# dat-rohit/distributed-neural-network

Hardware: AMD Instinct MI355X
Metric: images/sec (whole node) + epoch time, CIFAR-10 CNN bs=64 at 1/2/4/8 MI355X (higher is better)
Workload: dtype bf16; 1 GPU; model=reference CIFAR-10 CNN (models/model.py Network, 62,006 params), engine=HipEngine, pipelined_step=True, persistent_launch=True, launch=direct-aql, global_batch=64, per_gpu_batch=64, parallelism=dp1, sync=step-allreduce, optimizer=SGD lr=0.001 momentum=0.9, every step, safe_transport=0

## Files before the change

csrc/kernels/lenet_fused.hip:

```cpp
#include <algorithm>
#include <cstddef>
#include <string>

#include "pers_common.h"
#include "runtime/aql_dispatch.h"

namespace dnn {

constexpr int NT = 512;
constexpr int CODES_PER_SAMPLE = 6 * 196 + 400;

constexpr int L_REGA = 0;
constexpr int L_REGA_SZ = 96256;
constexpr int L_REGB = L_REGA + L_REGA_SZ;
constexpr int L_REGB_SZ = 44544;
constexpr int B_WF = 17472;
constexpr int L_P1 = L_REGB + L_REGB_SZ;
constexpr int L_CODE1 = L_P1 + 3360;
constexpr int L_A0 = L_CODE1 + 1184;
constexpr int L_A0B = L_A0 + 1600;
constexpr int L_CODE2 = L_A0B + 832;
constexpr int L_H1 = L_CODE2 + 400;
constexpr int L_H1B = L_H1 + 512;
constexpr int L_H2 = L_H1B + 256;
constexpr int L_H2B = L_H2 + 384;
constexpr int L_LOG = L_H2B + 192;
constexpr int L_DZ3 = L_LOG + 64;
constexpr int L_DZ3B = L_DZ3 + 64;
constexpr int L_DZ2 = L_DZ3B + 64;
constexpr int L_DZ2B = L_DZ2 + 384;
constexpr int L_DZ1 = L_DZ2B + 192;
constexpr int L_DZ1B = L_DZ1 + 512;
constexpr int L_DA0 = L_DZ1B + 256;
constexpr int L_IMG = L_DA0 + 1600;
constexpr int L_MISC = L_IMG + 3072;
constexpr int L_F1C = L_MISC + 64;
constexpr int LDS_TOTAL = L_F1C + 128;
static_assert(LDS_TOTAL <= 163840, "LDS budget");
static_assert(B_WF + 20480 <= L_REGB_SZ, "REGB sub-layout");

constexpr int A_R3 = 0;
constexpr int A_DY2 = 73728;
constexpr int DY2_CS = 176;
constexpr int A_DP1 = A_DY2 + 16 * DY2_CS * 2;
constexpr int A_RS = A_DP1 + 4704;
constexpr int A_DY1 = 0;
constexpr int DY1_CH = 1824;
constexpr int A_RS1 = A_DY1 + 6 * DY1_CH;
static_assert(A_RS + 1152 <= L_REGA_SZ, "REGA sub-layout");
static_assert(A_RS1 + 672 <= A_DP1, "phase F scratch must not overlap dP1");

__device__ __forceinline__ bf16 u8norm_bf16(uint32_t u) {
  return (bf16)__builtin_fmaf((float)u, (float)(2.0 / 255.0), -1.0f);
}

__device__ __forceinline__ void lds_barrier() {
  asm volatile("s_waitcnt lgkmcnt(0)\n\ts_barrier" ::: "memory");
}

__device__ __forceinline__ void dma16(const void* gsrc, uint32_t lds_base) {
  unsigned keep;
  asm volatile(
      "s_mov_b32 %0, m0\n\ts_mov_b32 m0, %2\n\ts_nop 0\n\tglobal_load_lds_dwordx4 %1, off\n\ts_mov_b32 m0, %0"
      : "=&s"(keep)
      : "v"(gsrc), "s"(lds_base)
      : "memory");
}

__device__ __forceinline__ uint32_t lds_addr(const void* p) {
  return (uint32_t)(uintptr_t)(const __attribute__((address_space(3))) unsigned char*)p;
}

template <typename T>
__device__ __forceinline__ void consume(T& v) {
  asm volatile("" : "+v"(v));
}

__device__ __forceinline__ f32x4 mfma32(bf16x8 a, bf16x8 b, f32x4 c) {
  return __builtin_amdgcn_mfma_f32_16x16x32_bf16(a, b, c, 0, 0, 0);
}

__device__ __forceinline__ bf16x8 zero8() {
  bf16x8 z;
#pragma unroll
  for (int j = 0; j < 8; ++j) z[j] = (bf16)0.f;
  return z;
}

__device__ __forceinline__ bf16x8 row0(const bf16* x, int k0, int fr) {
  const bf16x8 v = *reinterpret_cast<const bf16x8*>(x + k0);
  return fr == 0 ? v : zero8();
}

__device__ __forceinline__ bf16x8 tr_frag(const bf16* m, int ld, int k0, int n0, int kmax, int lane) {
  typedef __attribute__((address_space(3))) bf16x4* lp;
  const int l16 = lane & 15, q = l16 >> 2, p = l16 & 3, fg = lane >> 4;
  const int r0 = min(k0 + 8 * fg + q, kmax - 1), r1 = min(k0 + 8 * fg + 4 + q, kmax - 1);
  const bf16x4 lo = __builtin_amdgcn_ds_read_tr16_b64_v4bf16((lp)(m + r0 * ld + n0 + 4 * p));
  const bf16x4 hi = __builtin_amdgcn_ds_read_tr16_b64_v4bf16((lp)(m + r1 * ld + n0 + 4 * p));
  bf16x8 v;
#pragma unroll
  for (int j = 0; j < 4; ++j) { v[j] = lo[j]; v[4 + j] = hi[j]; }
  return v;
}

__device__ __forceinline__ void build_r1_part(const uint8_t* img, bf16x8* R1, int row, int q) {
  const uint32_t* src = reinterpret_cast<const uint32_t*>(img + row * 32);
  uint32_t w[4];
#pragma unroll
  for (int k = 0; k < 4; ++k) w[k] = src[min(2 * q + k, 7)];
  bf16 v[16];
#pragma unroll
  for (int k = 0; k < 16; ++k) {
    const uint32_t u = (w[k >> 2] >> (8 * (k & 3))) & 0xffu;
    const bf16 t = u8norm_bf16(u);
    v[k] = (8 * q + k < 32) ? t : (bf16)0.f;
  }
#pragma unroll
  for (int x = 0; x < 8; ++x) {
    if (8 * q + x < 29) {
// ... 69 lines not shown
constexpr int PIPE_CTR_STRIDE = 32;
static_assert(PIPE_BLOCKS == GRAD_REDUCE_BLOCKS, "the pipelined launch runs the whole grad_reduce");
static_assert(PIPE_C2_BLOCKS > 0, "conv2 keeps blocks of its own");
int pipe_reduce_blocks() { return PIPE_BLOCKS; }
int pipe_groups() { return PIPE_GROUPS; }

__device__ __forceinline__ int pipe_group_blocks(int grp) {
  return grp == PG_C1 ? PIPE_C1_BLOCKS : grp == PG_C2 ? PIPE_C2_BLOCKS : PIPE_MLP_BLOCKS;
}
__device__ __forceinline__ long pipe_ctr_index(int par, int grp) { return (long)(PIPE_GROUPS * par + grp) * PIPE_CTR_STRIDE; }
__device__ __forceinline__ long pipe_flag_index(int par, int grp, int b, int batch) {
  return ((long)(PIPE_GROUPS * par + grp) * batch + b) * PIPE_CTR_STRIDE;
}

__device__ __forceinline__ void pipe_reduce(const ReduceArgs& a, const PipeCtl& pc, int wg, long long* stamps) {
  const int half = threadIdx.x >> 8, m = 2 * wg + half, rtid = threadIdx.x & 255;
  if (wg == 0) {
    if (threadIdx.x < PIPE_GROUPS) pc.ctr[pipe_ctr_index(pc.par ^ 1, threadIdx.x)] = 0u;
    for (int i = threadIdx.x; i < PIPE_GROUPS * a.batch; i += blockDim.x)
      pc.flg[pipe_flag_index(pc.par ^ 1, i / a.batch, i % a.batch, a.batch)] = 0u;
  }
  int grp = -1;
  if (m < pc.nred) {
    int rblk = 0;
    if (pc.nred > 1) {
      if (m < PIPE_CONV_BLOCKS) { rblk = PIPE_MLP_BLOCKS + m; grp = m < PIPE_C1_BLOCKS ? PG_C1 : PG_C2; }
      else if (m == PIPE_CONV_BLOCKS) rblk = PIPE_MLP_BLOCKS + PIPE_CONV_BLOCKS;
      else { rblk = m - PIPE_CONV_BLOCKS - 1; grp = PG_MLP; }
    }
    WtSink sk;
    grad_reduce_body(a, sk, rblk, rtid);
  }
  if (stamps != nullptr && threadIdx.x == 0) stamps[16 + 4 * wg + 1] = (long long)__builtin_amdgcn_s_memrealtime();
  asm volatile("s_waitcnt vmcnt(0)" ::: "memory");
  __syncthreads();
  if ((rtid >> 6) == 0 && grp >= 0) {
    unsigned old = 0;
    if (rtid == 0)
      old = __hip_atomic_fetch_add(pc.ctr + pipe_ctr_index(pc.par, grp), 1u, __ATOMIC_RELAXED, __HIP_MEMORY_SCOPE_AGENT);
    old = __builtin_amdgcn_readfirstlane(old);
    if (stamps != nullptr && rtid == 0 && half == 0) stamps[16 + 4 * wg + 3] = (long long)__builtin_amdgcn_s_memrealtime();
    if (old == (unsigned)pipe_group_blocks(grp) - 1u)
      for (int b = rtid; b < a.batch; b += 64)
        __hip_atomic_store(pc.flg + pipe_flag_index(pc.par, grp, b, a.batch), 1u, __ATOMIC_RELAXED,
                           __HIP_MEMORY_SCOPE_AGENT);
  }
}

__device__ __forceinline__ void pipe_wait(const PipeCtl& pc, int grp, int b, int batch, long long* diag = nullptr,
                                          int also = -1, bool* also_set = nullptr, unsigned tgt = 1u) {
  const unsigned* f = pc.flg + pipe_flag_index(pc.par, grp, b, batch);
  const unsigned* g = pc.flg + pipe_flag_index(pc.par, also < 0 ? grp : also, b, batch);
  if (__hip_atomic_load(pc.err, __ATOMIC_RELAXED, __HIP_MEMORY_SCOPE_AGENT) != 0u) return;
  const long long t0 = wall_clock64();
  if (diag != nullptr) diag[0] = t0;
  long long polls = 0;
  while (true) {
    const unsigned v = __hip_atomic_load(f, __ATOMIC_RELAXED, __HIP_MEMORY_SCOPE_AGENT);
    const unsigned w = also >= 0 ? __hip_atomic_load(g, __ATOMIC_RELAXED, __HIP_MEMORY_SCOPE_AGENT) : 0u;
    if (diag != nullptr && polls < 12) {
      diag[4082 + 2 * polls] = (long long)__builtin_amdgcn_s_memrealtime();
      diag[4083 + 2 * polls] = v;
    }
    if (v >= tgt) {
      if (also_set != nullptr) *also_set = w >= tgt;
      break;
    }
    ++polls;
    if (diag != nullptr) diag[1] = polls;
    __builtin_amdgcn_s_sleep(2);
    if (wall_clock64() - t0 > pc.timeout_ticks) {
      __hip_atomic_store(pc.err, 1u, __ATOMIC_RELAXED, __HIP_MEMORY_SCOPE_SYSTEM);
      break;
    }
  }
}

constexpr int PERS_WG = (PIPE_BLOCKS + 1) / 2;
constexpr int PERS_CONV_WG = (PIPE_CONV_BLOCKS + 1 + 1) / 2;
constexpr int PERS_C1_WG = PIPE_C1_BLOCKS / 2;
static_assert((PIPE_CONV_BLOCKS + 1) % 2 == 0, "conv + bookkeeping blocks fill whole workgroups");
static_assert(PIPE_C1_BLOCKS % 2 == 0, "the conv1 group is whole workgroups");
static_assert(PERS_WG <= PERS_RROW, "one ready word per reduction workgroup in a sample's row");
int persist_ctl_bytes(int batch) { return (int)(pers_arrive_off(batch) + (long)PERS_WG * PERS_AROW * 4); }

__device__ __forceinline__ void pers_arrive(const PipeCtl& pc, int kind, int b, unsigned tag, int lane) {
  const int w0 = kind ? PERS_CONV_WG : 0, nw = kind ? PERS_WG - PERS_CONV_WG : PERS_CONV_WG;
  if (lane < nw) st_tag(pc.arrive + (long)(w0 + lane) * PERS_AROW + b, tag);
}

struct PersPoll {
  unsigned err, v;
};
__device__ __forceinline__ const unsigned* pers_ready_word(const PipeCtl& pc, int b, int lane) {
  return pc.flg + (long)b * PERS_RROW + min(lane, PERS_WG - 1);
}
__device__ __forceinline__ PersPoll pers_poll_issue(const PipeCtl& pc, int b, int lane) {
  return PersPoll{ld_tag(pc.err), ld_tag(pers_ready_word(pc, b, lane))};
}
__device__ __forceinline__ void pers_wait_ready(const PipeCtl& pc, int b, int lo, int hi, unsigned tgt, int lane,
                                                int also_lo = 0, int also_hi = 0, bool* also_set = nullptr,
                                                long long* diag = nullptr, bool has_pre = false, unsigned pre_err = 0u,
                                                unsigned pre_v = 0u) {
  const unsigned* row = pers_ready_word(pc, b, lane);
  unsigned ferr = pre_err, v = pre_v;
  if (!has_pre) {
    const PersPoll first = pers_poll_issue(pc, b, lane);
    ferr = first.err;
    v = first.v;
  }
  if (ferr != 0u) return;
  const long long t0 = wall_clock64();
  if (diag != nullptr && lane == 0) diag[0] = t0;
  long long polls = 0;
  while (true) {
    if (__all((lane < lo || lane >= hi) || tag_ge(v, tgt))) {
      if (also_set != nullptr) *also_set = __all((lane < also_lo || lane >= also_hi) || tag_ge(v, tgt));
      break;
    }
    ++polls;
    if (diag != nullptr && lane == 0) diag[1] = polls;
    __builtin_amdgcn_s_sleep(1);
    if (wall_clock64() - t0 > pc.timeout_ticks) {
      if (lane == 0) __hip_atomic_store(pc.err, 1u, __ATOMIC_RELAXED, __HIP_MEMORY_SCOPE_SYSTEM);
      break;
    }
    v = ld_tag(row);
  }
}

template <class F>
__device__ __forceinline__ bool pers_wait_c1_early_fc1(const PipeCtl& pc, int b, unsigned tgt, int lane,
                                                       F&& stream_all) {
  const unsigned* row = pers_ready_word(pc, b, lane);
  const PersPoll first = pers_poll_issue(pc, b, lane);
  if (first.err != 0u) return false;
  const long long t0 = wall_clock64();
  bool streamed = false;
  unsigned v = first.v;
  while (true) {
    if (__all(lane >= PERS_C1_WG || tag_ge(v, tgt))) break;
    if (!streamed && __all(lane < PERS_CONV_WG || tag_ge(v, tgt))) {
      stream_all();
      streamed = true;
    }
    __builtin_amdgcn_s_sleep(1);
    if (wall_clock64() - t0 > pc.timeout_ticks) {
      if (lane == 0) __hip_atomic_store(pc.err, 1u, __ATOMIC_RELAXED, __HIP_MEMORY_SCOPE_SYSTEM);
      break;
    }
    v = ld_tag(row);
  }
  return streamed;
}

template <int XNR>
__device__ __forceinline__ void pers_reduce(const ReduceArgs& a, const PipeCtl& pc, int wg, long long* stamps) {
  const int half = __builtin_amdgcn_readfirstlane(threadIdx.x >> 8), m = 2 * wg + half, rtid = threadIdx.x & 255,
            lane = threadIdx.x & 63;
  const bool bk = m == PIPE_CONV_BLOCKS;
  int rblk = 0;
  if (m < PIPE_CONV_BLOCKS) rblk = PIPE_MLP_BLOCKS + m;
  else if (!bk) rblk = m - PIPE_CONV_BLOCKS - 1;
  const unsigned g0 = __builtin_amdgcn_readfirstlane(ld_tag(pc.gen + blockIdx.x));
  const int gb = bk ? PIPE_MLP_BLOCKS + PIPE_CONV_BLOCKS : rblk;
  const unsigned xc0 = XNR > 1 ? __builtin_amdgcn_readfirstlane(a.xp_ctr[gb]) : 0u;
  if (bk && rtid < 64) bookkeeping_pers(a, pc, lane, -1);
  const unsigned* arr = pc.arrive + (long)wg * PERS_AROW;
  for (int t = 0; t < pc.nsteps; ++t) {
    if (threadIdx.x < 64) pers_wait_rows(pc, arr, a.batch, g0 + (unsigned)t + 1u, lane);
    const bool st = stamps != nullptr && threadIdx.x == 0 && t == pc.nsteps - 1;
    if (st) stamps[2400 + 4 * wg] = (long long)__builtin_amdgcn_s_memrealtime();
    __syncthreads();
    int tid_o = threadIdx.x;
    asm volatile("" : "+v"(tid_o));
    const int rtid_s = tid_o & 255;
    if (bk) {
      if (rtid < 64) bookkeeping_pers(a, pc, lane, t);
    } else if constexpr (XNR > 1) {
      const unsigned step = xc0 + (unsigned)t + 1u;
      const bool failed = __hip_atomic_load(a.xp_err, __ATOMIC_RELAXED, __HIP_MEMORY_SCOPE_SYSTEM) != 0u;
      XpSinkT<false, true> sk;
      sk.tag = (unsigned long long)step << 32;
      sk.stash = tid_o;
      sk.stride = NT;
      const bool publish = (a.xp_mode & 2) == 0 || gb % a.xp_nranks != a.xp_rank;
      sk.own = publish ? reinterpret_cast<unsigned long long*>(a.xp_region[a.xp_rank] + a.xp_gslot_off +
                                                               (step & 1u) * a.xp_gslot_bytes)
                       : nullptr;
      if (grad_reduce_body<XpSinkT<false, true>, true>(a, sk, rblk, rtid_s, t & 1)) {
        if ((a.xp_mode & 2) == 0) xp_exchange<XNR>(a, sk, step, failed, rblk, rtid_s);
        else xp_exchange_rsag<XNR>(a, sk, step, failed, rblk, rtid_s);
      }
    } else {
      WtSink sk;
      grad_reduce_body<WtSink, true>(a, sk, rblk, rtid_s, t & 1);
    }
    if (st) stamps[2401 + 4 * wg] = (long long)__builtin_amdgcn_s_memrealtime();
    const bool wst = stamps != nullptr && (threadIdx.x & 63) == 0 && t == pc.nsteps - 1 && wg < PERS_C1_WG;
    if (wst) stamps[2640 + 16 * wg + 2 * (threadIdx.x >> 6)] = (long long)__builtin_amdgcn_s_memrealtime();
    asm volatile("s_waitcnt vmcnt(0)" ::: "memory");
    if (wst) stamps[2641 + 16 * wg + 2 * (threadIdx.x >> 6)] = (long long)__builtin_amdgcn_s_memrealtime();
    __syncthreads();
    if (st) stamps[2402 + 4 * wg] = (long long)__builtin_amdgcn_s_memrealtime();
    if (threadIdx.x < 64)
      for (int b = lane; b < a.batch; b += 64) st_tag(pc.flg + (long)b * PERS_RROW + wg, g0 + (unsigned)t + 1u);
  }
  if (threadIdx.x == 0) st_tag(pc.gen + blockIdx.x, g0 + (unsigned)pc.nsteps);
  if constexpr (XNR > 1) {
    if (rtid == 0) a.xp_ctr[gb] = xc0 + (unsigned)pc.nsteps;
  }
}

template <bool WT>
struct WeightRd {
  const bf16* sh;
  const float* ms;
  __amdgpu_buffer_rsrc_t r;
  __device__ __forceinline__ WeightRd(const bf16* shadow, const float* master) : sh(shadow), ms(master) {
    if constexpr (WT) r = __builtin_amdgcn_make_buffer_rsrc(const_cast<bf16*>(shadow), 0, SH_TOTAL * 2, 0x00020000);
  }
  __device__ __forceinline__ bf16x8 w8(int e) const {
    if constexpr (WT) return __builtin_bit_cast(bf16x8, __builtin_amdgcn_raw_buffer_load_b128(r, e * 2, 0, 16));
    else return *reinterpret_cast<const bf16x8*>(sh + e);
  }
  __device__ __forceinline__ bf16x4 w4(int e) const {
    if constexpr (WT) return __builtin_bit_cast(bf16x4, __builtin_amdgcn_raw_buffer_load_b64(r, e * 2, 0, 16));
    else return *reinterpret_cast<const bf16x4*>(sh + e);
  }
  __device__ __forceinline__ float f(int i) const {
    if constexpr (WT)
      return __uint_as_float(__hip_atomic_load(reinterpret_cast<const unsigned*>(ms + i), __ATOMIC_RELAXED,
                                               __HIP_MEMORY_SCOPE_AGENT));
    else return ms[i];
  }
};

__device__ __forceinline__ void dma16_sc1(const void* gsrc, uint32_t lds_base) {
  unsigned keep;
  asm volatile(
      "s_mov_b32 %0, m0\n\ts_mov_b32 m0, %2\n\ts_nop 0\n\tglobal_load_lds_dwordx4 %1, off sc1\n\ts_mov_b32 m0, %0"
      : "=&s"(keep)
      : "v"(gsrc), "s"(lds_base)
      : "memory");
}
template <bool WT>
__device__ __forceinline__ void dma_w(const void* gsrc, uint32_t lds_base) {
  if constexpr (WT) dma16_sc1(gsrc, lds_base);
  else dma16(gsrc, lds_base);
}

__constant__ unsigned char kF1Col[80] = {73, 39, 201, 19, 35, 65, 56, 42, 30, 27, 59, 33, 38, 3, 25, 62, 74, 20, 17, 0, 57, 23, 72, 36, 13, 53, 10, 4, 22, 202, 18, 34, 54, 182, 67, 41, 68, 28, 2, 71, 31, 11, 55, 15, 40, 6, 9, 58, 49, 51, 37, 177, 43, 44, 12, 63, 21, 26, 24, 14, 60, 61, 48, 64, 50, 7, 70, 47, 46, 69, 45, 1, 8, 16, 32, 5, 66, 29, 178, 52};

template <bool TRAIN, bool STAGED = false, bool PIPE = false, bool PERS = false, int XNR = 0>
__global__ void __launch_bounds__(NT) __attribute__((amdgpu_waves_per_eu(1, 2))) lenet_fused_kernel(
    const uint8_t* __restrict__ images,
    const int32_t* __restrict__ labels,
    const int32_t* __restrict__ order,
    int order_len, int batch, int base_index,
    int32_t* __restrict__ state,
    const float* __restrict__ master,
    const bf16* __restrict__ shadow,
    float* __restrict__ a0_out, float* __restrict__ h1_out, float* __restrict__ h2_out,
    float* __restrict__ z1_out, float* __restrict__ z2_out, float* __restrict__ z3_out,
    float* __restrict__ slab_out, float* __restrict__ loss_out, int32_t* __restrict__ correct_out,
    long long* __restrict__ stamps,
    uint8_t* __restrict__ codes_out,
    const int32_t* __restrict__ next_ids,
    unsigned char* __restrict__ stage,
    const ReduceArgs ra,
    const PipeCtl pc) {
  static_assert(!PIPE || (TRAIN && STAGED), "the pipelined step is a staged training launch");
  static_assert(!PERS || PIPE, "the persistent launch is a PIPE grid");
  static_assert(XNR == 0 || PERS, "the in-launch exchange is a persistent-launch feature");
  extern __shared__ __attribute__((aligned(16))) unsigned char smem[];
  const bool btrace = stamps != nullptr && threadIdx.x == 0;
  if (btrace) {
    stamps[16 + 4 * blockIdx.x] = (long long)__builtin_amdgcn_s_memrealtime();
    stamps[16 + 4 * blockIdx.x + 3] = (long long)__builtin_amdgcn_s_getreg((20 << 0) | (0 << 6) | (3 << 11));
  }
  const int nrw = PIPE ? (pc.nred + 1) / 2 : 0;
  if constexpr (PIPE) {
    if ((int)blockIdx.x < nrw) {
      if constexpr (PERS) pers_reduce<XNR>(ra, pc, blockIdx.x, XNR > 1 ? nullptr : stamps);
      else pipe_reduce(ra, pc, blockIdx.x, stamps);
      if (btrace) stamps[16 + 4 * blockIdx.x + 2] = (long long)__builtin_amdgcn_s_memrealtime();
      return;
    }
  }
  const int b = (int)blockIdx.x - nrw;
  const WeightRd<PIPE> wr(shadow, master);
  uint4 carry_im = make_uint4(0, 0, 0, 0);
  int carry_lab = 0;
  const int nsteps = PERS ? pc.nsteps : 1;
  const unsigned g0 = PERS ? __builtin_amdgcn_readfirstlane(ld_tag(pc.gen + blockIdx.x)) : 0u;
  if (TRAIN && threadIdx.x < 80) smem[L_F1C + threadIdx.x] = kF1Col[threadIdx.x];
  int s = 0;
  do {
  int tid_opaque = threadIdx.x;
  if constexpr (PERS) asm volatile("" : "+v"(tid_opaque));
  const int tid = tid_opaque;
  const int lane = tid & 63;
  const int wave = tid >> 6;
  const int fr = lane & 15;
  const int fg = lane >> 4;
  const long rsh = PERS ? (long)(s & 1) * batch : 0;
  float* const a0_s = a0_out + rsh * A0_LD;
  float* const h1_s = h1_out + rsh * H1_LD;
  float* const h2_s = h2_out + rsh * H2_LD;
  float* const z1_s = z1_out + rsh * Z1_LD;
  float* const z2_s = z2_out + rsh * Z2_LD;
  float* const z3_s = z3_out + rsh * Z3_LD;
  float* const slab_s = slab_out + rsh * SLAB;
  float* const loss_s = loss_out + rsh;
  int32_t* const correct_s = correct_out + rsh;
  const int do_wait = PERS ? (s > 0 ? 1 : 0) : pc.wait;
  const unsigned wtgt = PERS ? g0 + (unsigned)s : 1u;
  const bool stamp = stamps != nullptr && (int)blockIdx.x == nrw && threadIdx.x == 0 && (!PERS || s == nsteps - 1);
  if (PERS && stamps != nullptr && (int)blockIdx.x == nrw && threadIdx.x == 0 && s < 1024)
    stamps[2048 + s] = (long long)__builtin_amdgcn_s_memrealtime();
#define STAMP(i) do { if (stamp) stamps[i] = (long long)__builtin_amdgcn_s_memrealtime(); } while (0)
  const bool wstamp = stamps != nullptr && (int)blockIdx.x == nrw && (threadIdx.x & 63) == 0 && (!PERS || s == nsteps - 1);
#define WSTAMP(base) do { if (wstamp) stamps[(base) + (threadIdx.x >> 6)] = (long long)__builtin_amdgcn_s_memrealtime(); } while (0)
  STAMP(0);

  int bvalid = 1, sample = 0;
  bool valid;
  uint4 st_im = make_uint4(0, 0, 0, 0);
  int st_label = 0;
  uint4* const stage_im = reinterpret_cast<uint4*>(stage);
  int32_t* const stage_lab = reinterpret_cast<int32_t*>(stage + (size_t)batch * IMG);
  constexpr bool staged = TRAIN && STAGED;
  if (TRAIN) {
    if constexpr (staged) {
      if (!PERS || s == 0) {
        st_im = stage_im[(size_t)b * (IMG / 16) + min(tid, IMG / 16 - 1)];
        st_label = stage_lab[b];
      }
    } else {
      sample = order[b];
    }
    if constexpr (PERS) bvalid = s == 0 ? *pc.bv_slot[0] : batch;
    else bvalid = PIPE ? *pc.bvalid : state[ST_BVALID];
    valid = b < bvalid;
  } else {
    const long gidx = (long)base_index + b;
    valid = gidx < order_len;
    sample = (int)gidx;
  }
  float my_loss = 0.f;
  int my_correct = 0;
  auto put_row = [&](float* p, float v) {
    if constexpr (PERS) st_wt(p, v);
    else *p = v;
  };
  auto pers_arrive_kind = [&](int kind) {
    if (PERS && (pc.flags & 256) && b == 0 && s == 1 && kind == 0 && tid == 0) {
      const long long t0 = wall_clock64();
      while (wall_clock64() - t0 < 3 * pc.timeout_ticks) __builtin_amdgcn_s_sleep(64);
    }
    asm volatile("s_waitcnt vmcnt(0)" ::: "memory");
    __syncthreads();
    if (wave == 0) pers_arrive(pc, kind, b, g0 + (unsigned)s + 1u, lane);
  };
  auto invalid_sample = [&]() {
    int ti = threadIdx.x, bo = b;
    asm volatile("" : "+v"(ti), "+v"(bo));
    for (int i = ti; i < A0_LD; i += NT) put_row(a0_s + (size_t)bo * A0_LD + i, 0.f);
    for (int i = ti; i < H1_LD; i += NT) {
      put_row(h1_s + (size_t)bo * H1_LD + i, 0.f);
      put_row(z1_s + (size_t)bo * Z1_LD + i, 0.f);
    }
    for (int i = ti; i < H2_LD; i += NT) {
      put_row(h2_s + (size_t)bo * H2_LD + i, 0.f);
      put_row(z2_s + (size_t)bo * Z2_LD + i, 0.f);
    }
    for (int i = ti; i < Z3_LD; i += NT) put_row(z3_s + (size_t)bo * Z3_LD + i, 0.f);
    for (int i = ti; i < SLAB; i += NT) put_row(slab_s + (size_t)bo * SLAB + i, 0.f);
    if (ti == 0) {
      put_row(loss_s + bo, 0.f);
      put_row(reinterpret_cast<float*>(correct_s + bo), 0.f);
    }
    if constexpr (PERS) {
      pers_arrive_kind(1);
      pers_arrive_kind(0);
    }
  };
  if (!valid) {
    if constexpr (PERS) {
      invalid_sample();
      continue;
    } else {
      if (TRAIN) {
        for (int i = tid; i < A0_LD; i += NT) a0_out[(size_t)b * A0_LD + i] = 0.f;
        for (int i = tid; i < H1_LD; i += NT) {
          h1_out[(size_t)b * H1_LD + i] = 0.f;
          z1_out[(size_t)b * Z1_LD + i] = 0.f;
        }
        for (int i = tid; i < H2_LD; i += NT) {
          h2_out[(size_t)b * H2_LD + i] = 0.f;
          z2_out[(size_t)b * Z2_LD + i] = 0.f;
        }
        for (int i = tid; i < Z3_LD; i += NT) z3_out[(size_t)b * Z3_LD + i] = 0.f;
        for (int i = tid; i < SLAB; i += NT) slab_out[(size_t)b * SLAB + i] = 0.f;
        if (tid == 0) { loss_out[b] = 0.f; correct_out[b] = 0; }
      }
      return;
    }
  }
  int label;
  const uint8_t* img = images + (size_t)sample * IMG;
  if constexpr (staged) label = st_label;
  else label = labels[sample];

  bf16* fc1s = reinterpret_cast<bf16*>(smem + L_REGA);
  bf16x8* R1 = reinterpret_cast<bf16x8*>(smem + L_REGB);
  bf16x8* R2 = reinterpret_cast<bf16x8*>(smem + L_REGB);
  bf16x8* WF = reinterpret_cast<bf16x8*>(smem + L_REGB + B_WF);
  bf16* P1 = reinterpret_cast<bf16*>(smem + L_P1);
  uint8_t* CODE1 = smem + L_CODE1;
  float* A0 = reinterpret_cast<float*>(smem + L_A0);
  bf16* A0B = reinterpret_cast<bf16*>(smem + L_A0B);
  uint8_t* CODE2 = smem + L_CODE2;
  float* H1 = reinterpret_cast<float*>(smem + L_H1);
  bf16* H1B = reinterpret_cast<bf16*>(smem + L_H1B);
  float* H2 = reinterpret_cast<float*>(smem + L_H2);
  bf16* H2B = reinterpret_cast<bf16*>(smem + L_H2B);
  float* LOG = reinterpret_cast<float*>(smem + L_LOG);
  float* DZ3 = reinterpret_cast<float*>(smem + L_DZ3);
  bf16* DZ3B = reinterpret_cast<bf16*>(smem + L_DZ3B);
  float* DZ2 = reinterpret_cast<float*>(smem + L_DZ2);
  bf16* DZ2B = reinterpret_cast<bf16*>(smem + L_DZ2B);
  float* DZ1 = reinterpret_cast<float*>(smem + L_DZ1);
  bf16* DZ1B = reinterpret_cast<bf16*>(smem + L_DZ1B);
  float* DA0 = reinterpret_cast<float*>(smem + L_DA0);
  uint8_t* IMGS = smem + L_IMG;

  uint4 im;
  if constexpr (staged) im = st_im;
  else im = reinterpret_cast<const uint4*>(img)[min(tid, 191)];
  bf16x8 bw1[4], bw2[8];
  float bias_c1 = 0.f, bias_c2 = 0.f;
  auto load_conv1_w = [&]() {
#pragma unroll
    for (int sk = 0; sk < 4; ++sk) bw1[sk] = wr.w8(SH_W1F + ((4 * sk + fg) * 16 + fr) * 8);
    bias_c1 = wr.f(OFF_C1B + min(fr >> 1, 5));
  };
  auto load_conv2_w = [&]() {
#pragma unroll
    for (int sk = 0; sk < 8; ++sk) bw2[sk] = wr.w8(SH_W2F + ((4 * sk + fg) * 16 + fr) * 8);
    bias_c2 = wr.f(OFF_C2B + fr);
  };
  auto consume_conv2_w = [&]() {
#pragma unroll
    for (int sk = 0; sk < 8; ++sk) consume(bw2[sk]);
    consume(bias_c2);
  };
  if constexpr (!PIPE) {
    load_conv1_w();
    load_conv2_w();
  }
  for (int i = tid; i < 6 * 14 * 20; i += NT) P1[i] = (bf16)0.f;
  if (tid < 16) A0B[400 + tid] = (bf16)0.f;
  else if (tid < 24) H1B[120 + tid - 16] = (bf16)0.f;
  else if (tid < 36) H2B[84 + tid - 24] = (bf16)0.f;
  else if (tid < 58) DZ3B[10 + tid - 36] = (bf16)0.f;
  else if (tid < 70) DZ2B[84 + tid - 58] = (bf16)0.f;
  else if (tid < 78) DZ1B[120 + tid - 70] = (bf16)0.f;
  if (PERS && s > 0) {
    if (tid >= 320) reinterpret_cast<uint4*>(IMGS)[tid - 320] = carry_im;
    if (tid == 320) *reinterpret_cast<int*>(smem + L_MISC) = carry_lab;
  } else {
    if (tid < 192) reinterpret_cast<uint4*>(IMGS)[tid] = im;
    if (PERS && tid == 0) *reinterpret_cast<int*>(smem + L_MISC) = label;
  }
  lds_barrier();
  if (PERS) label = *reinterpret_cast<const int*>(smem + L_MISC);
  STAMP(9);
  if (tid < 384) build_r1_part(IMGS, R1, r1_row(tid), r1_q(tid));
  unsigned c2_err = 0u, c2_v = 0u;
  int bv_pre = batch;
  if constexpr (PIPE) {
    if constexpr (PERS) {
      if (wave == 0) {
        bool early = false;
        if (do_wait && !(pc.flags & 3)) {
          early = pers_wait_c1_early_fc1(pc, b, wtgt, lane, [&]() {
            const uint4* f1src = reinterpret_cast<const uint4*>(shadow + OFF_F1W);
            const uint32_t base = __builtin_amdgcn_readfirstlane(lds_addr(smem + L_REGA));
            for (int i = 0; i < 94; ++i) dma_w<PIPE>(f1src + i * 64 + lane, base + (uint32_t)i * 1024u);
          });
        } else if (do_wait) {
          pers_wait_ready(pc, b, 0, PERS_C1_WG, wtgt, lane, 0, 0, nullptr, stamp ? stamps + 14 : nullptr);
        }
        if (lane == 0) reinterpret_cast<int*>(smem + L_MISC)[1] = early ? 1 : 0;
      }
    } else {
      if (tid == 0 && do_wait) pipe_wait(pc, PG_C1, b, batch, stamp ? stamps + 14 : nullptr, -1, nullptr, wtgt);
    }
    STAMP(12);
    lds_barrier();
    if constexpr (PERS) {
      if (do_wait) {
        const PersPoll p = pers_poll_issue(pc, b, lane);
        c2_err = p.err;
        c2_v = p.v;
      }
      if (s > 1) bv_pre = ld_sc1(pc.bv_slot[s & 1]);
    }
    load_conv1_w();
  } else {
#pragma unroll
    for (int sk = 0; sk < 4; ++sk) consume(bw1[sk]);
    consume(bias_c1);
    consume_conv2_w();
  }
  STAMP(11);
  auto stream_fc1 = [&]() {
    const uint4* f1src = reinterpret_cast<const uint4*>(shadow + OFF_F1W);
    const uint32_t base = __builtin_amdgcn_readfirstlane(lds_addr(smem + L_REGA));
#pragma unroll
    for (int k = 0; k < 12; ++k) {
      const int i = min(wave + 8 * k, 93);
      dma_w<PIPE>(f1src + i * 64 + lane, base + (uint32_t)__builtin_amdgcn_readfirstlane(i) * 1024u);
    }
  };
  if constexpr (!PIPE) {
    stream_fc1();
    lds_barrier();
  }
  bool fc1_out = !PIPE;
  if constexpr (PERS) fc1_out = reinterpret_cast<const int*>(smem + L_MISC)[1] != 0;
  int bv_late = bv_pre;
  STAMP(1);

  {
    float bias = 0.f;
    const int wl = fr >> 1, dy = fr & 1;
    auto a_index = [&](int t, int sk) {
      const int q = min(8 * t + wl, 195);
      const int y = 2 * (q / 14) + dy, x = 2 * (q % 14);
      const int pr = min(4 * sk + fg, 14);
      return (pr / 5 * 32 + y + pr % 5) * 29 + x;
    };
    auto epilogue = [&](int t, f32x4 acc) {
      float nb[4];
#pragma unroll
      for (int i = 0; i < 4; ++i)
        nb[i] = __int_as_float(__builtin_amdgcn_mov_dpp(__float_as_int(acc[i]), 0xB1, 0xf, 0xf, false));
      if (fr < 12 && dy == 0) {
        const int o = fr >> 1;
#pragma unroll
        for (int h = 0; h < 2; ++h) {
          const int qo = 8 * t + 2 * fg + h;
          if (qo < 196) {
            float best = acc[2 * h] + bias;
            int arg = 0;
            const float v1 = nb[2 * h] + bias, v2 = acc[2 * h + 1] + bias, v3 = nb[2 * h + 1] + bias;
            if (v1 > best) { best = v1; arg = 1; }
            if (v2 > best) { best = v2; arg = 2; }
            if (v3 > best) { best = v3; arg = 3; }
            P1[(o * 14 + qo / 14) * 20 + qo % 14] = (bf16)fmaxf(best, 0.f);
            CODE1[o * 196 + qo] = best > 0.f ? (uint8_t)arg : (uint8_t)4;
          }
        }
      }
    };
#pragma unroll
    for (int r = 0; r < 2; ++r) {
      const int t0 = r == 0 ? wave : wave + 16, t1 = r == 0 ? wave + 8 : 24;
      const bool two = r == 0 || wave == 0;
      bf16x8 a0[4], a1[4];
#pragma unroll
      for (int sk = 0; sk < 4; ++sk) {
        a0[sk] = R1[a_index(t0, sk)];
        if (two) a1[sk] = R1[a_index(t1, sk)];
      }
      __builtin_amdgcn_sched_barrier(0);
      f32x4 acc0 = {0.f, 0.f, 0.f, 0.f}, acc1 = {0.f, 0.f, 0.f, 0.f};
#pragma unroll
      for (int sk = 0; sk < 4; ++sk) {
        acc0 = mfma32(a0[sk], bw1[sk], acc0);
        if (two) acc1 = mfma32(a1[sk], bw1[sk], acc1);
      }
      if (r == 0) {
        asm volatile("" : "+v"(bias_c1));
        bias = fr < 12 ? bias_c1 : 0.f;
      }
      epilogue(t0, acc0);
      if (two) epilogue(t1, acc1);
      STAMP(1000 + 3 * r);
      WSTAMP(1010 + 10 * r);
      if (PIPE && r == 0) {
        int mlp = 0;
        if constexpr (PERS) {
          bool m = true;
          unsigned c2e = c2_err, c2v = c2_v;
          asm volatile("" : "+v"(c2e), "+v"(c2v) : "v"(acc0[0]));
          if (do_wait) pers_wait_ready(pc, b, PERS_C1_WG, PERS_CONV_WG, wtgt, lane, PERS_CONV_WG, PERS_WG, &m, nullptr, true,
                                       c2e, c2v);
          mlp = m && !(pc.flags & 1);
        } else if (lane == 0) {
          bool m = false;
          if (do_wait) pipe_wait(pc, PG_C2, b, batch, nullptr, (pc.flags & 1) ? -1 : PG_MLP, &m, wtgt);
          else m = true;
          mlp = m && !(pc.flags & 1);
        }
        if (PERS && s == 1) bv_late = ld_sc1(pc.bv_slot[s & 1]);
        STAMP(1001);
        WSTAMP(1040);
        if (!fc1_out && __builtin_amdgcn_readfirstlane(mlp)) {
          stream_fc1();
          fc1_out = true;
        }
        load_conv2_w();
        STAMP(1002);
      }
    }
  }
  if constexpr (PIPE) {
    if (!fc1_out) {
      if constexpr (PERS) {
        if (do_wait) pers_wait_ready(pc, b, PERS_CONV_WG, PERS_WG, wtgt, lane);
      } else {
        if (lane == 0 && do_wait) pipe_wait(pc, PG_MLP, b, batch, nullptr, -1, nullptr, wtgt);
      }
      consume_conv2_w();
      stream_fc1();
    }
    STAMP(13);
  }
  WSTAMP(1050);
  lds_barrier();
  if constexpr (PERS) {
    if (s > 0) {
      bvalid = bv_late;
      valid = b < bvalid;
      if (!valid) {
        asm volatile("s_waitcnt vmcnt(0)" ::: "memory");
        invalid_sample();
        continue;
      }
    }
  }

  STAMP(2);
  const int ncol = 16 * wave + fr;
  if (tid < 168) {
    const int row = tid >> 1, h = tid & 1;
    bf16 v[14];
#pragma unroll
    for (int k = 0; k < 14; ++k) v[k] = P1[row * 20 + 7 * h + k];
#pragma unroll
    for (int x = 0; x < 7; ++x) {
      if (7 * h + x < 13) {
        bf16x8 r;
#pragma unroll
        for (int j = 0; j < 8; ++j) r[j] = v[x + j];
        R2[row * 13 + 7 * h + x] = r;
      }
    }
  }
  bf16x8 w2f[4], w2t[3], w3t, w3f[3];
  float bias_f1 = wr.f(OFF_F1B + min(ncol, 119));
  {
    const int r2 = OFF_F2W + min(ncol, 83) * 120;
    if (wave < 6) {
#pragma unroll
      for (int ks = 0; ks < 4; ++ks) w2f[ks] = wr.w8(r2 + 32 * ks + 8 * fg);
      w3t = wr.w8(SH_W3T + min(ncol, 83) * 16 + 8 * fg);
    }
    if (wave == 0) {
      const int r3 = OFF_F3W + min(fr, 9) * 84;
#pragma unroll
      for (int ks = 0; ks < 3; ++ks) {
        const bf16x4 lo = wr.w4(r3 + 32 * ks + 8 * fg);
        const bf16x4 hi = wr.w4(r3 + 32 * ks + 8 * fg + 4);
#pragma unroll
        for (int j = 0; j < 4; ++j) { w3f[ks][j] = lo[j]; w3f[ks][4 + j] = hi[j]; }
      }
    }
  }
  float bias_f2 = 0.f, bias_f3 = 0.f;
// ... 336 lines not shown
        float tv = 0.f;
        if (x < 28) tv = cd[x >> 1] == (yb | (x & 1)) ? dv[x >> 1] : 0.f;
        rs += tv;
        r[j] = (bf16)tv;
      }
      drow[g8] = r;
    }
    RS1[c * 28 + y] = rs;
    static_assert(2 * (NT - 168) <= 768 && 768 - 2 * (NT - 168) <= 168, "R1 half-task split");
    if (tid < 768 - 2 * (NT - 168)) build_r1_half(IMGS, R1, 2 * (NT - 168) + tid);
  } else {
    if (staged && wave >= 5) {
      const int32_t* p = (PERS ? pc.nid_slot[s & 1] : next_ids) + b;
      asm volatile("" : "+v"(p));
      ns_next = PERS ? ld_sc1(p) : *p;
    }
    build_r1_half(IMGS, R1, tid - 168);
    build_r1_half(IMGS, R1, tid - 168 + (NT - 168));
  }
  lds_barrier();
  STAMP(10);
  if (staged && wave >= 5 && ns_next >= 0) {
    const int t = tid - 320;
    const uint4 v = reinterpret_cast<const uint4*>(images + (size_t)ns_next * IMG)[t];
    const int lab = t == 0 ? labels[ns_next] : 0;
    stage_im[(size_t)b * (IMG / 16) + t] = v;
    if (t == 0) stage_lab[b] = lab;
    if constexpr (PERS) {
      carry_im = v;
      carry_lab = lab;
    }
  }
  if (wave == 7) {
    const int c = min(lane >> 3, 5), part = lane & 7;
    float t = 0.f;
#pragma unroll
    for (int k = 0; k < 4; ++k) t += (part + 8 * k < 28) ? RS1[c * 28 + min(part + 8 * k, 27)] : 0.f;
    t = sum8(t);
    if (part == 0 && lane < 48) SLAB_PUT(SLAB_C1B + c, t);
  }
  if (wave < 5) {
    const int ent = smem[L_F1C + wave * 16 + fr];
    const int nc = ent & 127;
    const int c = nc / 25, ky = (nc % 25) / 5, kx = nc % 5;
    const unsigned char* arow = DY1 + fr * DY1_CH + fg * 16;
    const bf16x8* brow = R1 + (c * 32 + ky) * 29 + 8 * fg + kx;
    f32x4 acc = {0.f, 0.f, 0.f, 0.f};
#pragma unroll
    for (int g = 0; g < 4; ++g) {
      bf16x8 av[7], bv[7];
#pragma unroll
      for (int k = 0; k < 7; ++k) {
        av[k] = *reinterpret_cast<const bf16x8*>(arow + (7 * g + k) * 64);
        bv[k] = brow[(7 * g + k) * 29];
      }
      __builtin_amdgcn_sched_barrier(0);
#pragma unroll
      for (int k = 0; k < 7; ++k) acc = mfma32(av[k], bv[k], acc);
    }
    if (ent < 128) {
#pragma unroll
      for (int i = 0; i < 4; ++i) {
        const int o = 4 * fg + i;
        if (o < 6) SLAB_PUT(SLAB_C1W + o * 75 + nc, acc[i]);
      }
    }
  }
  if (codes_out != nullptr) {
    for (int i = tid; i < CODES_PER_SAMPLE; i += NT)
      codes_out[(size_t)b * CODES_PER_SAMPLE + i] = i < 6 * 196 ? CODE1[i] : CODE2[i - 6 * 196];
  }
  if (stamp) {
    __builtin_amdgcn_s_waitcnt(0);
    STAMP(7);
  }
  if constexpr (PERS) {
    pers_arrive_kind(0);
    if (stamp) stamps[2398] = (long long)__builtin_amdgcn_s_memrealtime();
  }
#undef STAMP
#undef WSTAMP
#undef SLAB_PUT
  } while (PERS && ++s < nsteps);
  if (PERS && threadIdx.x == 0) st_tag(pc.gen + blockIdx.x, g0 + (unsigned)nsteps);
  if (btrace) stamps[16 + 4 * blockIdx.x + 2] = (long long)__builtin_amdgcn_s_memrealtime();
}

}

namespace dnn {

void init_kernels() {
  static bool done = false;
  if (done) return;
  const void* kerns[] = {(const void*)lenet_fused_kernel<true, false>, (const void*)lenet_fused_kernel<true, true>,
                         (const void*)lenet_fused_kernel<false, false>, (const void*)lenet_fused_kernel<true, true, true>,
                         (const void*)lenet_fused_kernel<true, true, true, true>,
                         (const void*)lenet_fused_kernel<true, true, true, true, 8>};
  for (const void* k : kerns) HIP_CHECK(hipFuncSetAttribute(k, hipFuncAttributeMaxDynamicSharedMemorySize, LDS_TOTAL));
  init_kernels_f32();
  done = true;
}

void launch_fused_train(const uint8_t* images, const int32_t* labels, const int32_t* order, int order_len,
                        int batch, int32_t* state, const float* master, const bf16* shadow, float* a0,
                        float* h1, float* h2, float* z1, float* z2, float* z3, float* slab, float* loss,
                        int32_t* correct, long long* stamps, const int32_t* next_ids, unsigned char* stage,
                        hipStream_t stream, uint8_t* codes) {
  init_kernels();
  if (stage != nullptr && next_ids == nullptr) throw std::runtime_error("fused_train: staging needs next_ids");
  auto* kern = stage ? &lenet_fused_kernel<true, true> : &lenet_fused_kernel<true, false>;
  hipLaunchKernelGGL(kern, dim3(batch), dim3(NT), LDS_TOTAL, stream, images, labels, order, order_len, batch, 0, state,
                     master, shadow, a0, h1, h2, z1, z2, z3, slab, loss, correct, stamps, codes, next_ids, stage,
                     ReduceArgs{}, PipeCtl{});
  HIP_CHECK(hipGetLastError());
}

void launch_fused_train_pipe(const uint8_t* images, const int32_t* labels, int order_len, int batch,
                             const float* master, const bf16* shadow, float* a0, float* h1, float* h2, float* z1,
                             float* z2, float* z3, float* slab, float* loss, int32_t* correct, long long* stamps,
                             const int32_t* next_ids, unsigned char* stage, const ReduceArgs& red, const PipeCtl& pc,
                             hipStream_t stream) {
  init_kernels();
  if (stage == nullptr || next_ids == nullptr || pc.bvalid == nullptr || pc.ctr == nullptr || pc.err == nullptr ||
      pc.flg == nullptr)
    throw std::runtime_error(
        "fused_train_pipe: needs the stage, its next_ids / bvalid slot, the counters, flags and error word");
  if (!(pc.nred == PIPE_BLOCKS || pc.nred == 1) || (pc.wait && pc.nred != PIPE_BLOCKS) || (pc.par & ~1))
    throw std::runtime_error("fused_train_pipe: nred must be the whole reduction or the bookkeeping alone");
  if (!red.bookkeeping || red.batch != batch || red.xp_nranks != 0 || !red.fuse_sgd)
    throw std::runtime_error("fused_train_pipe: a local fused-SGD reduction with bookkeeping of this batch");
  if (pc.nred == PIPE_BLOCKS ? !(red.lo == 0 && red.hi >= ARENA) : !(red.lo == OFF_F1W && red.hi == OFF_F1W))
    throw std::runtime_error("fused_train_pipe: whole-arena reduction, or an empty range for the bookkeeping alone");
  if (batch < 1 || batch > 1024) throw std::runtime_error("fused_train_pipe: batch out of range");
  const int nrw = (pc.nred + 1) / 2;
  hipLaunchKernelGGL((lenet_fused_kernel<true, true, true>), dim3(nrw + batch), dim3(NT), LDS_TOTAL, stream, images,
                     labels, nullptr, order_len, batch, 0, red.state, master, shadow, a0, h1, h2, z1, z2, z3, slab,
                     loss, correct, stamps, nullptr, next_ids, stage, red, pc);
  HIP_CHECK(hipGetLastError());
}

constexpr int PERS_MARGIN = 8;
int persist_resident_workgroups() {
  static int resident = -1;
  if (resident < 0) {
    init_kernels();
    int dev = 0, cus = 0, per_cu = 0;
    HIP_CHECK(hipGetDevice(&dev));
    HIP_CHECK(hipDeviceGetAttribute(&cus, hipDeviceAttributeMultiprocessorCount, dev));
    HIP_CHECK(hipOccupancyMaxActiveBlocksPerMultiprocessor(
        &per_cu, reinterpret_cast<const void*>(lenet_fused_kernel<true, true, true, true>), NT, LDS_TOTAL));
    int per_cu_x = 0;
    HIP_CHECK(hipOccupancyMaxActiveBlocksPerMultiprocessor(
        &per_cu_x, reinterpret_cast<const void*>(lenet_fused_kernel<true, true, true, true, 8>), NT, LDS_TOTAL));
    resident = std::min(per_cu, per_cu_x) * cus;
  }
  return resident;
}
int persist_max_batch() {
  return std::max(0, std::min(persist_resident_workgroups() - PERS_WG - PERS_MARGIN, PERS_AROW));
}

struct PersKernargs {
  const uint8_t* images;
  const int32_t* labels;
  const int32_t* order;
  int order_len, batch, base_index;
// ... 78 lines not shown
```

Before: 4.136 million images/s.

## Hand off updated conv1 weights via tagged mailbox instead of ready flags

Adds a mailbox of 64-bit tag+value granules. The conv1 reduction workgroups write each SGD-updated conv1 weight and bias into it, and the persistent fused kernel polls it and scatters the values straight into an LDS copy of the conv1 filter layout. Most conv1 reduction workgroups skip the vmcnt drain, barrier and ready-flag publish, so the forward pass no longer waits on a full ready-flag round trip plus a reload from the shadow weights. The cost is extra LDS, more complex polling across all waves, and a new control-block region whose tag protocol must stay consistent.

```diff
diff --git a/csrc/kernels/lenet_fused.hip b/csrc/kernels/lenet_fused.hip
--- a/csrc/kernels/lenet_fused.hip
+++ b/csrc/kernels/lenet_fused.hip
@@ -2,7 +2,7 @@
 #include <cstddef>
 #include <string>
 
-#include "pers_common.h"
+#include "pers_handoff.h"
 #include "runtime/aql_dispatch.h"
 
 namespace dnn {
@@ -35,7 +35,9 @@
 constexpr int L_IMG = L_DA0 + 1600;
 constexpr int L_MISC = L_IMG + 3072;
 constexpr int L_F1C = L_MISC + 64;
-constexpr int LDS_TOTAL = L_F1C + 128;
+constexpr int L_W1F = L_F1C + 128;
+constexpr int L_B1 = L_W1F + 4096;
+constexpr int LDS_TOTAL = L_B1 + 32;
 static_assert(LDS_TOTAL <= 163840, "LDS budget");
 static_assert(B_WF + 20480 <= L_REGB_SZ, "REGB sub-layout");
 
@@ -271,7 +273,8 @@
 static_assert((PIPE_CONV_BLOCKS + 1) % 2 == 0, "conv + bookkeeping blocks fill whole workgroups");
 static_assert(PIPE_C1_BLOCKS % 2 == 0, "the conv1 group is whole workgroups");
 static_assert(PERS_WG <= PERS_RROW, "one ready word per reduction workgroup in a sample's row");
-int persist_ctl_bytes(int batch) { return (int)(pers_arrive_off(batch) + (long)PERS_WG * PERS_AROW * 4); }
+static_assert(HO_WG == PERS_WG, "pers_handoff.h's control block layout");
+int persist_ctl_bytes(int batch) { return (int)ho_ctl_bytes(batch); }
 
 __device__ __forceinline__ void pers_arrive(const PipeCtl& pc, int kind, int b, unsigned tag, int lane) {
   const int w0 = kind ? PERS_CONV_WG : 0, nw = kind ? PERS_WG - PERS_CONV_WG : PERS_CONV_WG;
@@ -343,6 +346,39 @@
   return streamed;
 }
 
+template <class F>
+__device__ __forceinline__ bool pers_wait_mbox(const PipeCtl& pc, int b, unsigned tgt, int lane, int w, bool watch_mlp,
+                                               bf16* w1f, float* b1, F&& stream_all) {
+  const unsigned long long* mw = ho_mbox(pc) + max(w, 0);
+  const unsigned* row = pers_ready_word(pc, b, lane);
+  bool pend = w >= 0;
+  const unsigned ferr = ld_tag(pc.err);
+  unsigned long long x = ld_gran(mw);
+  unsigned v = watch_mlp ? ld_tag(row) : 0u;
+  if (ferr != 0u) return false;
+  const long long t0 = wall_clock64();
+  bool streamed = false;
+  while (true) {
+    if (pend && (unsigned)(x >> 32) == tgt) {
+      ho_mbox_to_lds(w, __uint_as_float((unsigned)x), w1f, b1);
+      pend = false;
+    }
+    if (!__any(pend)) break;
+    if (watch_mlp && !streamed && __all(lane < PERS_CONV_WG || tag_ge(v, tgt))) {
+      stream_all();
+      streamed = true;
+    }
+    __builtin_amdgcn_s_sleep(1);
+    if (wall_clock64() - t0 > pc.timeout_ticks) {
+      if (lane == 0) __hip_atomic_store(pc.err, 1u, __ATOMIC_RELAXED, __HIP_MEMORY_SCOPE_SYSTEM);
+      break;
+    }
+    if (pend) x = ld_gran(mw);
+    if (watch_mlp && !streamed) v = ld_tag(row);
+  }
+  return streamed;
+}
+
 template <int XNR>
 __device__ __forceinline__ void pers_reduce(const ReduceArgs& a, const PipeCtl& pc, int wg, long long* stamps) {
   const int half = __builtin_amdgcn_readfirstlane(threadIdx.x >> 8), m = 2 * wg + half, rtid = threadIdx.x & 255,
@@ -356,6 +392,7 @@
   const unsigned xc0 = XNR > 1 ? __builtin_amdgcn_readfirstlane(a.xp_ctr[gb]) : 0u;
   if (bk && rtid < 64) bookkeeping_pers(a, pc, lane, -1);
   const unsigned* arr = pc.arrive + (long)wg * PERS_AROW;
+  constexpr bool MBOX = XNR == 0 && HO_MBOX;
   for (int t = 0; t < pc.nsteps; ++t) {
     if (threadIdx.x < 64) pers_wait_rows(pc, arr, a.batch, g0 + (unsigned)t + 1u, lane);
     const bool st = stamps != nullptr && threadIdx.x == 0 && t == pc.nsteps - 1;
@@ -366,6 +403,9 @@
     const int rtid_s = tid_o & 255;
     if (bk) {
       if (rtid < 64) bookkeeping_pers(a, pc, lane, t);
+    } else if (MBOX && m < PIPE_C1_BLOCKS) {
+      MboxSink sk{ho_mbox(pc), g0 + (unsigned)t + 1u};
+      conv_task<MboxSink, true>(m * RT + rtid_s, a, sk, t & 1);
     } else if constexpr (XNR > 1) {
       const unsigned step = xc0 + (unsigned)t + 1u;
       const bool failed = __hip_atomic_load(a.xp_err, __ATOMIC_RELAXED, __HIP_MEMORY_SCOPE_SYSTEM) != 0u;
@@ -388,6 +428,11 @@
     if (st) stamps[2401 + 4 * wg] = (long long)__builtin_amdgcn_s_memrealtime();
     const bool wst = stamps != nullptr && (threadIdx.x & 63) == 0 && t == pc.nsteps - 1 && wg < PERS_C1_WG;
     if (wst) stamps[2640 + 16 * wg + 2 * (threadIdx.x >> 6)] = (long long)__builtin_amdgcn_s_memrealtime();
+    if (MBOX && wg < PERS_C1_WG - 1) {
+      if (wst) stamps[2641 + 16 * wg + 2 * (threadIdx.x >> 6)] = (long long)__builtin_amdgcn_s_memrealtime();
+      if (st) stamps[2402 + 4 * wg] = (long long)__builtin_amdgcn_s_memrealtime();
+      continue;
+    }
     asm volatile("s_waitcnt vmcnt(0)" ::: "memory");
     if (wst) stamps[2641 + 16 * wg + 2 * (threadIdx.x >> 6)] = (long long)__builtin_amdgcn_s_memrealtime();
     __syncthreads();
@@ -484,6 +529,8 @@
   const int nsteps = PERS ? pc.nsteps : 1;
   const unsigned g0 = PERS ? __builtin_amdgcn_readfirstlane(ld_tag(pc.gen + blockIdx.x)) : 0u;
   if (TRAIN && threadIdx.x < 80) smem[L_F1C + threadIdx.x] = kF1Col[threadIdx.x];
+  constexpr bool MBOX = PERS && XNR == 0 && HO_MBOX;
+  if (MBOX && threadIdx.x < 256) reinterpret_cast<uint4*>(smem + L_W1F)[threadIdx.x] = make_uint4(0, 0, 0, 0);
   int s = 0;
   do {
   int tid_opaque = threadIdx.x;
@@ -517,6 +564,8 @@
   bool valid;
   uint4 st_im = make_uint4(0, 0, 0, 0);
   int st_label = 0;
+  bf16x8 w1_pre = zero8();
+  float b1_pre = 0.f;
   uint4* const stage_im = reinterpret_cast<uint4*>(stage);
   int32_t* const stage_lab = reinterpret_cast<int32_t*>(stage + (size_t)batch * IMG);
   constexpr bool staged = TRAIN && STAGED;
@@ -525,6 +574,10 @@
       if (!PERS || s == 0) {
         st_im = stage_im[(size_t)b * (IMG / 16) + min(tid, IMG / 16 - 1)];
         st_label = stage_lab[b];
+      }
+      if (MBOX && s == 0) {
+        w1_pre = wr.w8(SH_W1F + min(tid, 255) * 8);
+        b1_pre = wr.f(OFF_C1B + min(tid, 5));
       }
     } else {
       sample = order[b];
@@ -631,9 +684,15 @@
   bf16x8 bw1[4], bw2[8];
   float bias_c1 = 0.f, bias_c2 = 0.f;
   auto load_conv1_w = [&]() {
-#pragma unroll
-    for (int sk = 0; sk < 4; ++sk) bw1[sk] = wr.w8(SH_W1F + ((4 * sk + fg) * 16 + fr) * 8);
-    bias_c1 = wr.f(OFF_C1B + min(fr >> 1, 5));
+    if constexpr (MBOX) {
+#pragma unroll
+      for (int sk = 0; sk < 4; ++sk) bw1[sk] = reinterpret_cast<const bf16x8*>(smem + L_W1F)[(4 * sk + fg) * 16 + fr];
+      bias_c1 = reinterpret_cast<const float*>(smem + L_B1)[min(fr >> 1, 5)];
+    } else {
+#pragma unroll
+      for (int sk = 0; sk < 4; ++sk) bw1[sk] = wr.w8(SH_W1F + ((4 * sk + fg) * 16 + fr) * 8);
+      bias_c1 = wr.f(OFF_C1B + min(fr >> 1, 5));
+    }
   };
   auto load_conv2_w = [&]() {
 #pragma unroll
@@ -670,7 +729,23 @@
   unsigned c2_err = 0u, c2_v = 0u;
   int bv_pre = batch;
   if constexpr (PIPE) {
-    if constexpr (PERS) {
+    if constexpr (MBOX) {
+      bf16* const w1l = reinterpret_cast<bf16*>(smem + L_W1F);
+      float* const b1l = reinterpret_cast<float*>(smem + L_B1);
+      bool early = false;
+      if (do_wait) {
+        const int w = wave == 0 ? (lane < HO_MBOX_ELEMS - 448 ? 448 + lane : -1) : tid - 64;
+        early = pers_wait_mbox(pc, b, wtgt, lane, w, wave == 0 && !(pc.flags & 3), w1l, b1l, [&]() {
+          const uint4* f1src = reinterpret_cast<const uint4*>(shadow + OFF_F1W);
+          const uint32_t base = __builtin_amdgcn_readfirstlane(lds_addr(smem + L_REGA));
+          for (int i = 0; i < 94; ++i) dma_w<PIPE>(f1src + i * 64 + lane, base + (uint32_t)i * 1024u);
+        });
+      } else {
+        if (tid < 256) reinterpret_cast<bf16x8*>(w1l)[tid] = w1_pre;
+        if (tid < 6) b1l[tid] = b1_pre;
+      }
+      if (tid == 0) reinterpret_cast<int*>(smem + L_MISC)[1] = early ? 1 : 0;
+    } else if constexpr (PERS) {
       if (wave == 0) {
         bool early = false;
         if (do_wait && !(pc.flags & 3)) {
@@ -786,8 +861,8 @@
           bool m = true;
           unsigned c2e = c2_err, c2v = c2_v;
           asm volatile("" : "+v"(c2e), "+v"(c2v) : "v"(acc0[0]));
-          if (do_wait) pers_wait_ready(pc, b, PERS_C1_WG, PERS_CONV_WG, wtgt, lane, PERS_CONV_WG, PERS_WG, &m, nullptr, true,
-                                       c2e, c2v);
+          if (do_wait) pers_wait_ready(pc, b, MBOX ? PERS_C1_WG - 1 : PERS_C1_WG, PERS_CONV_WG, wtgt, lane, PERS_CONV_WG,
+                                       PERS_WG, &m, nullptr, true, c2e, c2v);
           mlp = m && !(pc.flags & 1);
         } else if (lane == 0) {
           bool m = false;
@@ -1290,7 +1365,11 @@
 #undef WSTAMP
 #undef SLAB_PUT
   } while (PERS && ++s < nsteps);
-  if (PERS && threadIdx.x == 0) st_tag(pc.gen + blockIdx.x, g0 + (unsigned)nsteps);
+  if (PERS && threadIdx.x == 0) {
+    int bi = blockIdx.x;
+    asm volatile("" : "+v"(bi));
+    st_tag(pc.gen + bi, g0 + (unsigned)nsteps);
+  }
   if (btrace) stamps[16 + 4 * blockIdx.x + 2] = (long long)__builtin_amdgcn_s_memrealtime();
 }
 
diff --git a/csrc/kernels/pers_handoff.h b/csrc/kernels/pers_handoff.h
--- /dev/null
+++ b/csrc/kernels/pers_handoff.h
@@ -0,0 +1,64 @@
+#pragma once
+#include "pers_common.h"
+
+#ifndef DNN_HANDOFF
+#define DNN_HANDOFF 2
+#endif
+
+namespace dnn {
+
+constexpr bool HO_MBOX = (DNN_HANDOFF & 2) != 0;
+
+constexpr int HO_WG = (PIPE_BLOCKS + 1) / 2;
+constexpr int HO_MBOX_ELEMS = SLAB_C2W;
+constexpr int HO_MBOX_WORDS = 512;
+static_assert(HO_MBOX_ELEMS <= HO_MBOX_WORDS, "the mailbox holds conv1");
+
+__host__ __device__ constexpr long ho_mbox_off(int batch) { return pers_arrive_off(batch) + 4L * HO_WG * PERS_AROW; }
+__host__ __device__ constexpr long ho_ctl_bytes(int batch) {
+  return ho_mbox_off(batch) + (HO_MBOX ? 8L * HO_MBOX_WORDS : 0L);
+}
+static_assert(ho_mbox_off(1) % 8 == 0 && ho_mbox_off(2) % 8 == 0, "granules are naturally aligned");
+
+__device__ __forceinline__ unsigned long long* ho_mbox(const PipeCtl& pc) {
+  return reinterpret_cast<unsigned long long*>(pc.arrive + (long)HO_WG * PERS_AROW);
+}
+
+__device__ __forceinline__ unsigned long long ld_gran(const unsigned long long* p) {
+  return __hip_atomic_load(p, __ATOMIC_RELAXED, __HIP_MEMORY_SCOPE_AGENT);
+}
+__device__ __forceinline__ void st_gran(unsigned long long* p, unsigned tag, float v) {
+  __hip_atomic_store(p, ((unsigned long long)tag << 32) | __float_as_uint(v), __ATOMIC_RELAXED,
+                     __HIP_MEMORY_SCOPE_AGENT);
+}
+
+struct MboxSink {
+  unsigned long long* mbox;
+  unsigned tag;
+  __device__ __forceinline__ void put(int, int e, float g, float p_old, float m_old, const ReduceArgs& a) {
+    g *= a.grad_scale;
+    float p, m;
+    sgd_update(g, p_old, m_old, a.lr, a.momentum, p, m);
+    int w = -1;
+    if (e >= OFF_C1W && e < OFF_C1W + 450) w = SLAB_C1W + (e - OFF_C1W);
+    else if (e >= OFF_C1B && e < OFF_C1B + 6) w = SLAB_C1B + (e - OFF_C1B);
+    if (w >= 0) st_gran(mbox + w, tag, p);
+    a.mom[e] = m;
+    if (is_bias(e)) st_wt(a.master + e, p);
+    else a.master[e] = p;
+    write_shadow_wt(a.shadow, e, p);
+  }
+};
+
+__device__ __forceinline__ void ho_mbox_to_lds(int w, float p, bf16* w1f, float* bias) {
+  if (w < SLAB_C1B) {
+    const bf16 v = (bf16)p;
+    const int n = w / 75, rem = w - 75 * n, c = rem / 25, ky = (rem % 25) / 5, kx = rem % 5;
+    w1f[((c * 5 + ky) * 16 + 2 * n) * 8 + kx] = v;
+    w1f[((c * 5 + ky) * 16 + 2 * n + 1) * 8 + kx + 1] = v;
+  } else {
+    bias[w - SLAB_C1B] = p;
+  }
+}
+
+}
```

New measurement: 4.172 million images/s (median of 6 runs). Within noise of the previous version (+0.9%).
